# DreamScene-Project/DreamScene

Hardware: AMD Instinct MI355X
Metric: fwd+bwd views/s @1024x1024, 500000 Gaussians (higher is better)
Workload: dtype f32

## Files before the change

### dreamscene_amd/csrc/radix_sort.h

```cpp
#pragma once
#include "gsr_common.h"
#include <type_traits>

namespace {

constexpr int kSortThreads = 256;
constexpr int kItemsLarge = 16;
constexpr int kItemsSmall = 4;
constexpr int kRadixBits = 8;
constexpr int kRadix = 1 << kRadixBits;

template <typename T>
__device__ __forceinline__ T* batch_ptr(T* p, size_t bstride) {
  typedef typename std::conditional<std::is_const<T>::value, const char, char>::type B;
  return p ? reinterpret_cast<T*>(reinterpret_cast<B*>(p) + (size_t)blockIdx.y * bstride) : p;
}
#define GSR_LDS_ORDER() asm volatile("" ::: "memory")

__device__ __forceinline__ uint64_t eff_count(const uint64_t* n_dev, uint64_t cap) {
  if (!n_dev) return cap;
  const uint64_t n = *n_dev;
  return n < cap ? n : cap;
}

template <int ITEMS>
__device__ __forceinline__ uint64_t sort_index(uint32_t blk, int wave, int item, int lane) {
  return (uint64_t)blk * (kSortThreads * ITEMS) + (uint64_t)(wave * (64 * ITEMS) + item * 64 + lane);
}

__device__ __forceinline__ unsigned long long match_digit(uint32_t d, bool valid) {
  unsigned long long m = __ballot(valid);
#pragma unroll
  for (int b = 0; b < kRadixBits; ++b) {
    const bool bit = (d >> b) & 1u;
    const unsigned long long bal = __ballot(bit);
    m &= bit ? bal : ~bal;
  }
  return m;
}

template <int ITEMS, bool DROP>
__global__ void __launch_bounds__(kSortThreads)
k_radix_hist(const uint32_t* __restrict__ keys, const uint64_t* __restrict__ n_dev, uint64_t cap, int shift,
             uint32_t nblk, uint32_t* __restrict__ hist, size_t bstride) {
  keys = batch_ptr(keys, bstride); n_dev = batch_ptr(n_dev, bstride); hist = batch_ptr(hist, bstride);
  __shared__ uint32_t h[kRadix];
  const int tid = threadIdx.x, lane = tid & 63, wave = tid >> 6;
  const uint64_t n = eff_count(n_dev, cap);
  h[tid] = 0;
  __syncthreads();
  if ((uint64_t)blockIdx.x * (kSortThreads * ITEMS) < n) {
#pragma unroll 4
    for (int it = 0; it < ITEMS; ++it) {
      const uint64_t e = sort_index<ITEMS>(blockIdx.x, wave, it, lane);
      bool valid = e < n;
      const uint32_t kk = valid ? keys[e] : 0u;
      if (DROP) valid = valid && (kk != 0xFFFFFFFFu);
      const uint32_t d = (kk >> shift) & (kRadix - 1);
      const unsigned long long m = match_digit(d, valid);
      if (valid && lane == __ffsll((long long)m) - 1) atomicAdd(&h[d], (uint32_t)__popcll(m));
    }
  }
  __syncthreads();
  hist[(uint64_t)tid * nblk + blockIdx.x] = h[tid];
}

template <int THREADS>
__device__ __forceinline__ void radix_scan_body(uint32_t* __restrict__ hist, uint32_t nblk_stride, uint32_t* __restrict__ totals,
                                                const uint64_t* __restrict__ n_items, uint32_t per_block, size_t bstride) {
  hist = batch_ptr(hist, bstride); totals = batch_ptr(totals, bstride); n_items = batch_ptr(n_items, bstride);
  uint32_t nblk = nblk_stride;
  if (n_items) {
    const uint64_t used = (*n_items + per_block - 1) / per_block;
    if (used < nblk) nblk = (uint32_t)used;
  }
  constexpr int NW = THREADS / 64;
  __shared__ uint32_t wave_tot[NW];
  __shared__ uint32_t carry_s;
  const int tid = threadIdx.x, lane = tid & 63, wave = tid >> 6;
  uint32_t* row = hist + (uint64_t)blockIdx.x * nblk_stride;
  if (tid == 0) carry_s = 0;
  __syncthreads();
  constexpr uint32_t kPer = 4;
  for (uint32_t base = 0; base < nblk; base += THREADS * kPer) {
    uint32_t x[kPer];
    uint32_t s = 0;
    const uint32_t first = base + tid * kPer;
#pragma unroll
    for (uint32_t k = 0; k < kPer; ++k) {
      x[k] = (first + k < nblk) ? row[first + k] : 0u;
      s += x[k];
    }
    uint32_t inc = s;
#pragma unroll
    for (int o = 1; o < 64; o <<= 1) {
      const uint32_t t = (uint32_t)__shfl_up((int)inc, o, 64);
      if (lane >= o) inc += t;
    }
    if (lane == 63) wave_tot[wave] = inc;
    __syncthreads();
    uint32_t woff = 0;
#pragma unroll
    for (int w = 0; w < NW; ++w) woff += (w < wave) ? wave_tot[w] : 0u;
    const uint32_t carry = carry_s;
    uint32_t run = carry + woff + inc - s;
#pragma unroll
    for (uint32_t k = 0; k < kPer; ++k) {
      if (first + k < nblk) row[first + k] = run;
      run += x[k];
    }
    __syncthreads();
    if (tid == THREADS - 1) carry_s = carry + woff + inc;
    __syncthreads();
  }
  if (tid == 0) totals[blockIdx.x] = carry_s;
}
__global__ void __launch_bounds__(256) k_radix_scan(uint32_t* __restrict__ hist, uint32_t nblk_stride,
                                                    uint32_t* __restrict__ totals,
                                                    const uint64_t* __restrict__ n_items, uint32_t per_block,
                                                    size_t bstride) {
  radix_scan_body<256>(hist, nblk_stride, totals, n_items, per_block, bstride);
}
__global__ void __launch_bounds__(1024) k_radix_scan_wide(uint32_t* __restrict__ hist, uint32_t nblk_stride,
                                                          uint32_t* __restrict__ totals,
                                                          const uint64_t* __restrict__ n_items, uint32_t per_block,
                                                          size_t bstride) {
  radix_scan_body<1024>(hist, nblk_stride, totals, n_items, per_block, bstride);
}

template <bool IOTA, int ITEMS, bool DROP>
__global__ void __launch_bounds__(kSortThreads)
k_radix_scatter(const uint32_t* __restrict__ keys_in, const uint32_t* __restrict__ vals_in,
                uint32_t* __restrict__ keys_out, uint32_t* __restrict__ vals_out, const uint64_t* __restrict__ n_dev,
                uint64_t cap, int shift, uint32_t nblk, const uint32_t* __restrict__ hist,
                const uint32_t* __restrict__ totals, uint64_t* __restrict__ n_out, size_t bstride) {
  keys_in = batch_ptr(keys_in, bstride); vals_in = batch_ptr(vals_in, bstride);
  keys_out = batch_ptr(keys_out, bstride); vals_out = batch_ptr(vals_out, bstride);
  n_dev = batch_ptr(n_dev, bstride); hist = batch_ptr(hist, bstride); totals = batch_ptr(totals, bstride);
  n_out = batch_ptr(n_out, bstride);
  __shared__ uint32_t wh[4][kRadix];
  __shared__ uint32_t dbase[kRadix];
  __shared__ uint32_t wtot[4];
  const int tid = threadIdx.x, lane = tid & 63, wave = tid >> 6;
  const uint64_t n = eff_count(n_dev, cap);
  if ((uint64_t)blockIdx.x * (kSortThreads * ITEMS) >= n) {
    if (DROP && n_out && blockIdx.x == 0 && tid == 0) *n_out = 0;
    return;
  }
#pragma unroll
  for (int w = 0; w < 4; ++w) wh[w][tid] = 0;
  {
    const uint32_t x = totals[tid];
    uint32_t inc = x;
#pragma unroll
    for (int o = 1; o < 64; o <<= 1) {
      const uint32_t t = (uint32_t)__shfl_up((int)inc, o, 64);
      if (lane >= o) inc += t;
    }
    if (lane == 63) wtot[wave] = inc;
    __syncthreads();
    uint32_t woff = 0;
    for (int w = 0; w < wave; ++w) woff += wtot[w];
    dbase[tid] = woff + inc - x;
    if (DROP && n_out && blockIdx.x == 0 && tid == kSortThreads - 1) *n_out = (uint64_t)(woff + inc);
  }
  __syncthreads();
  uint32_t* mywh = wh[wave];
  uint32_t key[ITEMS];
  uint32_t val[ITEMS];
  uint32_t rank[ITEMS];
  const unsigned long long lt = (1ull << lane) - 1ull;
#pragma unroll
  for (int it = 0; it < ITEMS; ++it) {
    const uint64_t e = sort_index<ITEMS>(blockIdx.x, wave, it, lane);
    const bool valid = e < n;
    key[it] = valid ? keys_in[e] : 0xFFFFFFFFu;
    val[it] = IOTA ? (uint32_t)e : (valid ? vals_in[e] : 0u);
  }
  const auto is_valid = [&](int it) {
    const uint64_t e = sort_index<ITEMS>(blockIdx.x, wave, it, lane);
    return (e < n) && (!DROP || key[it] != 0xFFFFFFFFu);
  };
#pragma unroll
  for (int it = 0; it < ITEMS; ++it) {
    const bool valid = is_valid(it);
    const uint32_t d = (key[it] >> shift) & (kRadix - 1);
    const unsigned long long m = match_digit(d, valid);
    const int leader = __ffsll((long long)m) - 1;
    uint32_t old = 0;
    if (valid && lane == leader) {
      old = mywh[d];
      mywh[d] = old + (uint32_t)__popcll(m);
    }
    old = (uint32_t)__shfl((int)old, valid ? leader : lane, 64);
    rank[it] = old + (uint32_t)__popcll(m & lt);
    GSR_LDS_ORDER();
  }
  __syncthreads();
  {
    uint32_t run = dbase[tid] + hist[(uint64_t)tid * nblk + blockIdx.x];
#pragma unroll
    for (int w = 0; w < 4; ++w) {
      const uint32_t c = wh[w][tid];
      wh[w][tid] = run;
      run += c;
    }
  }
  __syncthreads();
#pragma unroll
  for (int it = 0; it < ITEMS; ++it) {
    if (is_valid(it)) {
      const uint32_t d = (key[it] >> shift) & (kRadix - 1);
      const uint32_t pos = wh[wave][d] + rank[it];
      keys_out[pos] = key[it];
      vals_out[pos] = val[it];
    }
  }
}

#ifndef GSR_OS_ITEMS_SMALL
#define GSR_OS_ITEMS_SMALL 16
#endif
constexpr int kOsItemsSmall = GSR_OS_ITEMS_SMALL;
constexpr int kOsMaxPasses = 4;
#ifndef GSR_OS_HIST_TILE
#define GSR_OS_HIST_TILE 2048
#endif
constexpr uint32_t kOsHistTile = GSR_OS_HIST_TILE;
constexpr uint32_t kOsTableOff = kOsMaxPasses * kRadix + 16;
constexpr uint32_t kOsSkipFlag = kOsMaxPasses * kRadix + 8;
constexpr uint32_t kOsEarlyN = kOsMaxPasses * kRadix + 10;
constexpr uint64_t kOsMaxN = 1ull << 28;

typedef __attribute__((address_space(1))) uint32_t gsr_gu32;
__device__ __forceinline__ gsr_gu32* gsr_global(uint32_t* p) { return (gsr_gu32*)(uintptr_t)p; }

__host__ __device__ inline uint32_t os_tiles(uint64_t n, int items) {
  const uint64_t t = (uint64_t)kSortThreads * items;
  return (uint32_t)((n + t - 1) / t);
}
__host__ inline size_t os_state_words(uint64_t n, int items) { return (size_t)kOsTableOff + (size_t)kRadix * os_tiles(n, items); }

template <bool DROP>
__global__ void __launch_bounds__(kSortThreads)
k_os_hist(const uint32_t* __restrict__ keys, const uint64_t* __restrict__ n_dev, uint64_t cap, int passes,
          uint32_t* __restrict__ os, size_t bstride, const uint32_t* __restrict__ wrect) {
  keys = batch_ptr(keys, bstride); n_dev = batch_ptr(n_dev, bstride); os = batch_ptr(os, bstride);
  wrect = batch_ptr(wrect, bstride);
  __shared__ uint32_t h[kOsMaxPasses][kRadix];
  __shared__ uint32_t wsum[kSortThreads / 64];
  const int tid = threadIdx.x, lane = tid & 63;
  const uint64_t n = eff_count(n_dev, cap);
  const uint64_t base = (uint64_t)blockIdx.x * kOsHistTile;
  if (base >= n) return;
#pragma unroll
  for (int p = 0; p < kOsMaxPasses; ++p) h[p][tid] = 0;
  __syncthreads();
  constexpr int kPer = kOsHistTile / kSortThreads;
  uint32_t kk[kPer];
  uint32_t weight = 0;
#pragma unroll
  for (int it = 0; it < kPer; ++it) {
    const uint64_t e = base + (uint64_t)(it * kSortThreads + tid);
    kk[it] = e < n ? keys[e] : 0xFFFFFFFFu;
    if (wrect && e < n && (!DROP || kk[it] != 0xFFFFFFFFu)) {
      const uint32_t r = wrect[e];
      weight += (((r >> 16) & 255u) + 1u) * ((r >> 24) + 1u);
    }
  }
  if (wrect) {
#pragma unroll
    for (int o = 32; o > 0; o >>= 1) weight += (uint32_t)__shfl_xor((int)weight, o, 64);
    if (lane == 0) wsum[tid >> 6] = weight;
  }
#pragma unroll
  for (int it = 0; it < kPer; ++it) {
    const uint64_t e = base + (uint64_t)(it * kSortThreads + tid);
    const bool valid = (e < n) && (!DROP || kk[it] != 0xFFFFFFFFu);
    const unsigned long long vm = __ballot(valid);
    if (vm == 0ull) continue;
    const uint32_t k = kk[it];
    if (valid) {
      atomicAdd(&h[0][k & (kRadix - 1)], 1u);
      if (passes > 1) atomicAdd(&h[1][(k >> kRadixBits) & (kRadix - 1)], 1u);
    }
    if (passes > 2) {
      const int first = __ffsll((long long)vm) - 1;
      const uint32_t hi = k >> (2 * kRadixBits), hi0 = (uint32_t)__shfl((int)hi, first, 64);
      if (__ballot(valid && hi != hi0) == 0ull) {
        if (lane == first) {
          atomicAdd(&h[2][hi0 & (kRadix - 1)], (uint32_t)__popcll(vm));
          if (passes > 3) atomicAdd(&h[3][hi0 >> kRadixBits], (uint32_t)__popcll(vm));
        }
      } else if (valid) {
        atomicAdd(&h[2][hi & (kRadix - 1)], 1u);
        if (passes > 3) atomicAdd(&h[3][hi >> kRadixBits], 1u);
      }
    }
  }
  __syncthreads();
  for (int p = 0; p < passes; ++p) {
    const uint32_t c = h[p][tid];
    if (c) atomicAdd(&os[p * kRadix + tid], c);
  }
  if (wrect && tid == 0) {
    const uint64_t w = ((uint64_t)wsum[0] + wsum[1]) + ((uint64_t)wsum[2] + wsum[3]);
    if (w) atomicAdd(reinterpret_cast<unsigned long long*>(os + kOsEarlyN), (unsigned long long)w);
  }
}

#ifndef GSR_OS_WINDOW
#define GSR_OS_WINDOW 16
#endif
constexpr int kOsWindow = GSR_OS_WINDOW;
__device__ __forceinline__ uint32_t os_look_back(gsr_gu32* table, uint32_t tile, int col, uint32_t tagA, uint32_t tagI) {
  uint32_t excl = 0;
  int p = (int)tile - 1;
  for (;;) {
    uint32_t w[kOsWindow];
#pragma unroll
    for (int j = 0; j < kOsWindow; ++j)
      w[j] = (p - j >= 0) ? __hip_atomic_load(table + (size_t)(p - j) * kRadix + col, __ATOMIC_RELAXED, __HIP_MEMORY_SCOPE_AGENT)
                          : 0u;
    bool done = false, stalled = false;
#pragma unroll
    for (int j = 0; j < kOsWindow; ++j) {
      if (done || stalled) continue;
      const uint32_t tag = w[j] & 0xF0000000u;
      if (tag == tagI) { excl += w[j] & 0x0FFFFFFFu; done = true; }
      else if (tag == tagA) { excl += w[j] & 0x0FFFFFFFu; --p; }
      else stalled = true;
    }
    if (done) return excl;
    if (stalled) __builtin_amdgcn_s_sleep(1);
  }
}

#ifdef GSR_OS_TRACE
__device__ unsigned long long* g_os_trace = nullptr;
#define GSR_OS_STAMP(k) do { if (threadIdx.x == 0 && g_os_trace) \
    g_os_trace[(((size_t)pass * 4 + blockIdx.y) * 4096 + blockIdx.x) * 8 + (k)] = wall_clock64(); } while (0)
#else
#define GSR_OS_STAMP(k) do { } while (0)
#endif

template <bool IOTA, int ITEMS, bool DROP>
__global__ void __launch_bounds__(kSortThreads)
k_os_pass(const uint32_t* __restrict__ keys_in, const uint32_t* __restrict__ vals_in, uint32_t* __restrict__ keys_out,
          uint32_t* __restrict__ vals_out, const uint64_t* __restrict__ n_dev, uint64_t cap, int pass,
          uint32_t* __restrict__ os, uint64_t* __restrict__ n_out, size_t bstride, const int may_skip,
          uint64_t* __restrict__ early_out) {
  keys_in = batch_ptr(keys_in, bstride); vals_in = batch_ptr(vals_in, bstride);
  keys_out = batch_ptr(keys_out, bstride); vals_out = batch_ptr(vals_out, bstride);
  n_dev = batch_ptr(n_dev, bstride); os = batch_ptr(os, bstride); n_out = batch_ptr(n_out, bstride);
  constexpr uint32_t T = kSortThreads * ITEMS;
  __shared__ uint32_t wh[4][kRadix];
  __shared__ uint32_t gbase[kRadix];
  __shared__ uint32_t skey[T], sval[T];
  __shared__ uint32_t wtot[4];
  __shared__ uint32_t s_tile, s_ntile;
  const int tid = threadIdx.x, lane = tid & 63, wave = tid >> 6;
  const int shift = pass * kRadixBits;
  const uint64_t n = eff_count(n_dev, cap);
  if constexpr (!DROP) {
    const uint32_t x = os[pass * kRadix + tid];
    if (__syncthreads_or((uint64_t)x == n && n > 0)) {
      if (may_skip) {
        if (blockIdx.x == 0 && tid == 0) os[kOsSkipFlag] = 1u;
        return;
      }
#pragma unroll
      for (int it = 0; it < ITEMS; ++it) {
        const uint64_t e = sort_index<ITEMS>(blockIdx.x, wave, it, lane);
        if (e < n) {
          keys_out[e] = keys_in[e];
          vals_out[e] = IOTA ? (uint32_t)e : vals_in[e];
        }
      }
      return;
    }
  }
  GSR_OS_STAMP(0);
  if (tid == 0) s_tile = atomicAdd(&os[kOsMaxPasses * kRadix + pass], 1u);
#pragma unroll
  for (int w = 0; w < 4; ++w) wh[w][tid] = 0;
  __syncthreads();
  const uint32_t tile = s_tile;
  if (early_out && tile == 0 && tid == 0)
    __hip_atomic_store(early_out + blockIdx.y, *reinterpret_cast<const uint64_t*>(os + kOsEarlyN), __ATOMIC_RELAXED,
                       __HIP_MEMORY_SCOPE_SYSTEM);
  if ((uint64_t)tile * T >= n) {
    if (DROP && n_out && tile == 0 && tid == 0) *n_out = 0;
    return;
  }
  uint32_t dbase;
  {
    const uint32_t x = os[pass * kRadix + tid];
    uint32_t inc = x;
#pragma unroll
    for (int o = 1; o < 64; o <<= 1) {
      const uint32_t t = (uint32_t)__shfl_up((int)inc, o, 64);
      if (lane >= o) inc += t;
    }
    if (lane == 63) wtot[wave] = inc;
    __syncthreads();
    uint32_t woff = 0;
    for (int w = 0; w < wave; ++w) woff += wtot[w];
    dbase = woff + inc - x;
    if (DROP && n_out && tile == 0 && tid == kSortThreads - 1) *n_out = (uint64_t)(woff + inc);
  }
  GSR_OS_STAMP(1);
#ifdef GSR_OS_TRACE
  if (threadIdx.x == 0 && g_os_trace) g_os_trace[(((size_t)pass * 4 + blockIdx.y) * 4096 + blockIdx.x) * 8 + 7] = tile;
#endif
  uint32_t* mywh = wh[wave];
  uint32_t key[ITEMS], val[ITEMS], rank[ITEMS];
  const unsigned long long lt = (1ull << lane) - 1ull;
#pragma unroll
  for (int it = 0; it < ITEMS; ++it) {
    const uint64_t e = sort_index<ITEMS>(tile, wave, it, lane);
    const bool valid = e < n;
    key[it] = valid ? keys_in[e] : 0xFFFFFFFFu;
    val[it] = IOTA ? (uint32_t)e : (valid ? vals_in[e] : 0u);
  }
  const auto is_valid = [&](int it) {
    const uint64_t e = sort_index<ITEMS>(tile, wave, it, lane);
    return (e < n) && (!DROP || key[it] != 0xFFFFFFFFu);
  };
#pragma unroll
  for (int it = 0; it < ITEMS; ++it) {
    const bool valid = is_valid(it);
    const uint32_t d = (key[it] >> shift) & (kRadix - 1);
    const unsigned long long m = match_digit(d, valid);
    const int leader = __ffsll((long long)m) - 1;
    uint32_t old = 0;
    if (valid && lane == leader) {
      old = mywh[d];
      mywh[d] = old + (uint32_t)__popcll(m);
    }
    old = (uint32_t)__shfl((int)old, valid ? leader : lane, 64);
    rank[it] = old + (uint32_t)__popcll(m & lt);
    GSR_LDS_ORDER();
  }
  __syncthreads();
  GSR_OS_STAMP(2);
  uint32_t cnt;
  {
    uint32_t run = 0;
#pragma unroll
    for (int w = 0; w < 4; ++w) {
      const uint32_t c = wh[w][tid];
      wh[w][tid] = run;
      run += c;
    }
    cnt = run;
  }
  gsr_gu32* table = gsr_global(os + kOsTableOff);
  const uint32_t tagA = (uint32_t)(2 * pass + 1) << 28, tagI = (uint32_t)(2 * pass + 2) << 28;
  uint32_t excl = 0;
  if (tile == 0) {
    __hip_atomic_store(table + tid, tagI | cnt, __ATOMIC_RELAXED, __HIP_MEMORY_SCOPE_AGENT);
  } else {
    __hip_atomic_store(table + (size_t)tile * kRadix + tid, tagA | cnt, __ATOMIC_RELAXED, __HIP_MEMORY_SCOPE_AGENT);
    excl = os_look_back(table, tile, tid, tagA, tagI);
    __hip_atomic_store(table + (size_t)tile * kRadix + tid, tagI | (excl + cnt), __ATOMIC_RELAXED, __HIP_MEMORY_SCOPE_AGENT);
  }
  GSR_OS_STAMP(3);
  uint32_t lstart;
  {
    uint32_t inc = cnt;
#pragma unroll
    for (int o = 1; o < 64; o <<= 1) {
      const uint32_t t = (uint32_t)__shfl_up((int)inc, o, 64);
      if (lane >= o) inc += t;
    }
    __syncthreads();
    if (lane == 63) wtot[wave] = inc;
    __syncthreads();
    uint32_t woff = 0;
    for (int w = 0; w < wave; ++w) woff += wtot[w];
    lstart = woff + inc - cnt;
    if (tid == kSortThreads - 1) s_ntile = woff + inc;
  }
#pragma unroll
  for (int w = 0; w < 4; ++w) wh[w][tid] += lstart;
  gbase[tid] = dbase + excl - lstart;
  __syncthreads();
#pragma unroll
  for (int it = 0; it < ITEMS; ++it) {
    if (is_valid(it)) {
      const uint32_t d = (key[it] >> shift) & (kRadix - 1);
      const uint32_t lp = wh[wave][d] + rank[it];
      skey[lp] = key[it];
      sval[lp] = val[it];
    }
  }
  __syncthreads();
  GSR_OS_STAMP(4);
  const uint32_t ntile = s_ntile;
  for (uint32_t i = tid; i < ntile; i += kSortThreads) {
    const uint32_t k = skey[i];
    const uint32_t pos = gbase[(k >> shift) & (kRadix - 1)] + i;
    keys_out[pos] = k;
    vals_out[pos] = sval[i];
  }
  GSR_OS_STAMP(5);
}

__host__ inline size_t align256(size_t x) { return (x + 255) & ~(size_t)255; }

uint32_t sort_blocks(uint64_t n, int items) {
  const uint64_t t = (uint64_t)kSortThreads * items;
  return (uint32_t)((n + t - 1) / t);
}

__host__ inline size_t sort_hist_bytes(uint64_t n, int items_legacy, int items_os) {
  const size_t legacy = (size_t)kRadix * sort_blocks(n, items_legacy) * 4;
  const size_t os = os_state_words(n, items_os) * 4;
  return align256(legacy > os ? legacy : os);
}

template <int ITEMS>
int radix_sort_u32_legacy(uint32_t* k0, uint32_t* v0, uint32_t* k1, uint32_t* v1, const uint64_t* n_dev, uint64_t cap,
                          int bits, bool iota, uint64_t* n_compact, uint32_t* hist, uint32_t* totals, hipStream_t stream,
                          int batch = 1, size_t bstride = 0);

template <int ITEMS, int OS_ITEMS>
int radix_sort_u32(uint32_t* k0, uint32_t* v0, uint32_t* k1, uint32_t* v1, const uint64_t* n_dev, uint64_t cap,
                   int bits, bool iota, uint64_t* n_compact, uint32_t* hist, uint32_t* totals, hipStream_t stream,
                   int batch = 1, size_t bstride = 0, bool state_cleared = false, bool last_pass_may_skip = false,
                   const uint32_t* early_rects = nullptr, uint64_t* early_out = nullptr) {
  const int passes = (bits + kRadixBits - 1) / kRadixBits;
  if (cap >= kOsMaxN || passes > kOsMaxPasses)
    return radix_sort_u32_legacy<ITEMS>(k0, v0, k1, v1, n_dev, cap, bits, iota, n_compact, hist, totals, stream, batch, bstride);
  const uint32_t ntile = os_tiles(cap, OS_ITEMS), nhist = (uint32_t)((cap + kOsHistTile - 1) / kOsHistTile);
  const dim3 grid(ntile, (uint32_t)batch), grid_h(nhist ? nhist : 1, (uint32_t)batch);
  if (!state_cleared &&
      gsr_zero_async(hist, os_state_words(cap, OS_ITEMS) * 4, stream, bstride, (uint32_t)batch) != hipSuccess) return passes & 1;
  const bool drop = iota && n_compact;
  if (!drop) { early_rects = nullptr; early_out = nullptr; }
  if (!early_out) early_rects = nullptr;
  if (drop)
    hipLaunchKernelGGL((k_os_hist<true>), grid_h, dim3(kSortThreads), 0, stream, k0, n_dev, cap, passes, hist, bstride,
                       early_rects);
  else
    hipLaunchKernelGGL((k_os_hist<false>), grid_h, dim3(kSortThreads), 0, stream, k0, n_dev, cap, passes, hist, bstride,
                       (const uint32_t*)nullptr);
  uint32_t *ka = k0, *va = v0, *kb = k1, *vb = v1;
  for (int p = 0; p < passes; ++p) {
    if (p == 0 && drop) {
      hipLaunchKernelGGL((k_os_pass<true, OS_ITEMS, true>), grid, dim3(kSortThreads), 0, stream, ka, va, kb, vb, n_dev, cap, p,
                         hist, n_compact, bstride, 0, early_rects ? early_out : (uint64_t*)nullptr);
      n_dev = n_compact;
    } else if (p == 0 && iota) {
      hipLaunchKernelGGL((k_os_pass<true, OS_ITEMS, false>), grid, dim3(kSortThreads), 0, stream, ka, va, kb, vb, n_dev, cap, p,
                         hist, (uint64_t*)nullptr, bstride, 0, (uint64_t*)nullptr);
    } else {
      hipLaunchKernelGGL((k_os_pass<false, OS_ITEMS, false>), grid, dim3(kSortThreads), 0, stream, ka, va, kb, vb, n_dev, cap, p,
                         hist, (uint64_t*)nullptr, bstride, (last_pass_may_skip && p == passes - 1 && p > 0) ? 1 : 0,
                         (uint64_t*)nullptr);
    }
    uint32_t* t = ka; ka = kb; kb = t;
    t = va; va = vb; vb = t;
  }
  return passes & 1;
}

template <int ITEMS>
int radix_sort_u32_legacy(uint32_t* k0, uint32_t* v0, uint32_t* k1, uint32_t* v1, const uint64_t* n_dev, uint64_t cap,
                   int bits, bool iota, uint64_t* n_compact, uint32_t* hist, uint32_t* totals, hipStream_t stream,
                   int batch, size_t bstride) {
  const uint32_t nblk = sort_blocks(cap, ITEMS);
  const int passes = (bits + kRadixBits - 1) / kRadixBits;
  const dim3 grid(nblk, (uint32_t)batch), grid_scan(kRadix, (uint32_t)batch);
  uint32_t *ka = k0, *va = v0, *kb = k1, *vb = v1;
  for (int p = 0; p < passes; ++p) {
    const int shift = p * kRadixBits;
    if (iota && p == 0 && n_compact) {
      hipLaunchKernelGGL((k_radix_hist<ITEMS, true>), grid, dim3(kSortThreads), 0, stream, ka, n_dev, cap, shift, nblk,
                         hist, bstride);
      hipLaunchKernelGGL(k_radix_scan, grid_scan, dim3(256), 0, stream, hist, nblk, totals, (const uint64_t*)nullptr, 1u,
                         bstride);
      hipLaunchKernelGGL((k_radix_scatter<true, ITEMS, true>), grid, dim3(kSortThreads), 0, stream, ka, va, kb, vb, n_dev,
                         cap, shift, nblk, hist, totals, n_compact, bstride);
      n_dev = n_compact;
    } else {
      hipLaunchKernelGGL((k_radix_hist<ITEMS, false>), grid, dim3(kSortThreads), 0, stream, ka, n_dev, cap, shift, nblk,
                         hist, bstride);
      hipLaunchKernelGGL(k_radix_scan, grid_scan, dim3(256), 0, stream, hist, nblk, totals, (const uint64_t*)nullptr, 1u,
                         bstride);
      if (iota && p == 0)
        hipLaunchKernelGGL((k_radix_scatter<true, ITEMS, false>), grid, dim3(kSortThreads), 0, stream, ka, va, kb, vb,
                           n_dev, cap, shift, nblk, hist, totals, (uint64_t*)nullptr, bstride);
      else
        hipLaunchKernelGGL((k_radix_scatter<false, ITEMS, false>), grid, dim3(kSortThreads), 0, stream, ka, va, kb, vb,
                           n_dev, cap, shift, nblk, hist, totals, (uint64_t*)nullptr, bstride);
    }
    uint32_t* t = ka; ka = kb; kb = t;
    t = va; va = vb; vb = t;
  }
  return passes & 1;
}

}
```

Baseline: 5121.

## Publish onesweep tile counts early and widen histogram blocks for batched sorts

The onesweep pass kernel now loads its keys first and builds per-tile digit counts in shared memory with atomics. It publishes the aggregate to the look-back table before the full per-wave ranking, so later tiles spin less on the decoupled look-back. The histogram kernel is templated on thread count and tile size, and batched sorts (batch>=2) use 1024-thread blocks over 8192-element tiles. This cuts block count and global atomics, at the cost of an extra LDS atomic pass per tile and more shared memory.

```diff
diff --git a/dreamscene_amd/csrc/radix_sort.h b/dreamscene_amd/csrc/radix_sort.h
--- a/dreamscene_amd/csrc/radix_sort.h
+++ b/dreamscene_amd/csrc/radix_sort.h
@@ -227,6 +227,12 @@
 #define GSR_OS_HIST_TILE 2048
 #endif
 constexpr uint32_t kOsHistTile = GSR_OS_HIST_TILE;
+#ifndef GSR_OS_HIST_WIDE
+#define GSR_OS_HIST_WIDE 1
+#endif
+constexpr int kOsHistWideThreads = 1024;
+constexpr uint32_t kOsHistWideTile = 8192;
+__host__ inline bool os_hist_wide(int batch) { return GSR_OS_HIST_WIDE && batch >= 2; }
 constexpr uint32_t kOsTableOff = kOsMaxPasses * kRadix + 16;
 constexpr uint32_t kOsSkipFlag = kOsMaxPasses * kRadix + 8;
 constexpr uint32_t kOsEarlyN = kOsMaxPasses * kRadix + 10;
@@ -241,27 +247,29 @@
 }
 __host__ inline size_t os_state_words(uint64_t n, int items) { return (size_t)kOsTableOff + (size_t)kRadix * os_tiles(n, items); }
 
-template <bool DROP>
-__global__ void __launch_bounds__(kSortThreads)
+template <bool DROP, int THREADS = kSortThreads, uint32_t TILE = kOsHistTile>
+__global__ void __launch_bounds__(THREADS)
 k_os_hist(const uint32_t* __restrict__ keys, const uint64_t* __restrict__ n_dev, uint64_t cap, int passes,
           uint32_t* __restrict__ os, size_t bstride, const uint32_t* __restrict__ wrect) {
   keys = batch_ptr(keys, bstride); n_dev = batch_ptr(n_dev, bstride); os = batch_ptr(os, bstride);
   wrect = batch_ptr(wrect, bstride);
   __shared__ uint32_t h[kOsMaxPasses][kRadix];
-  __shared__ uint32_t wsum[kSortThreads / 64];
+  __shared__ uint32_t wsum[THREADS / 64];
   const int tid = threadIdx.x, lane = tid & 63;
   const uint64_t n = eff_count(n_dev, cap);
-  const uint64_t base = (uint64_t)blockIdx.x * kOsHistTile;
+  const uint64_t base = (uint64_t)blockIdx.x * TILE;
   if (base >= n) return;
-#pragma unroll
-  for (int p = 0; p < kOsMaxPasses; ++p) h[p][tid] = 0;
-  __syncthreads();
-  constexpr int kPer = kOsHistTile / kSortThreads;
+  if (tid < kRadix) {
+#pragma unroll
+    for (int p = 0; p < kOsMaxPasses; ++p) h[p][tid] = 0;
+  }
+  __syncthreads();
+  constexpr int kPer = TILE / THREADS;
   uint32_t kk[kPer];
   uint32_t weight = 0;
 #pragma unroll
   for (int it = 0; it < kPer; ++it) {
-    const uint64_t e = base + (uint64_t)(it * kSortThreads + tid);
+    const uint64_t e = base + (uint64_t)(it * THREADS + tid);
     kk[it] = e < n ? keys[e] : 0xFFFFFFFFu;
     if (wrect && e < n && (!DROP || kk[it] != 0xFFFFFFFFu)) {
       const uint32_t r = wrect[e];
@@ -275,7 +283,7 @@
   }
 #pragma unroll
   for (int it = 0; it < kPer; ++it) {
-    const uint64_t e = base + (uint64_t)(it * kSortThreads + tid);
+    const uint64_t e = base + (uint64_t)(it * THREADS + tid);
     const bool valid = (e < n) && (!DROP || kk[it] != 0xFFFFFFFFu);
     const unsigned long long vm = __ballot(valid);
     if (vm == 0ull) continue;
@@ -299,18 +307,25 @@
     }
   }
   __syncthreads();
-  for (int p = 0; p < passes; ++p) {
-    const uint32_t c = h[p][tid];
-    if (c) atomicAdd(&os[p * kRadix + tid], c);
+  if (tid < kRadix) {
+    for (int p = 0; p < passes; ++p) {
+      const uint32_t c = h[p][tid];
+      if (c) atomicAdd(&os[p * kRadix + tid], c);
+    }
   }
   if (wrect && tid == 0) {
-    const uint64_t w = ((uint64_t)wsum[0] + wsum[1]) + ((uint64_t)wsum[2] + wsum[3]);
+    uint64_t w = 0;
+#pragma unroll
+    for (int i = 0; i < THREADS / 64; ++i) w += wsum[i];
     if (w) atomicAdd(reinterpret_cast<unsigned long long*>(os + kOsEarlyN), (unsigned long long)w);
   }
 }
 
 #ifndef GSR_OS_WINDOW
 #define GSR_OS_WINDOW 16
+#endif
+#ifndef GSR_OS_EARLY_PUBLISH
+#define GSR_OS_EARLY_PUBLISH 1
 #endif
 constexpr int kOsWindow = GSR_OS_WINDOW;
 __device__ __forceinline__ uint32_t os_look_back(gsr_gu32* table, uint32_t tile, int col, uint32_t tagA, uint32_t tagI) {
@@ -359,6 +374,9 @@
   __shared__ uint32_t skey[T], sval[T];
   __shared__ uint32_t wtot[4];
   __shared__ uint32_t s_tile, s_ntile;
+#if GSR_OS_EARLY_PUBLISH
+  __shared__ uint32_t tcnt[kRadix];
+#endif
   const int tid = threadIdx.x, lane = tid & 63, wave = tid >> 6;
   const int shift = pass * kRadixBits;
   const uint64_t n = eff_count(n_dev, cap);
@@ -384,6 +402,9 @@
   if (tid == 0) s_tile = atomicAdd(&os[kOsMaxPasses * kRadix + pass], 1u);
 #pragma unroll
   for (int w = 0; w < 4; ++w) wh[w][tid] = 0;
+#if GSR_OS_EARLY_PUBLISH
+  tcnt[tid] = 0;
+#endif
   __syncthreads();
   const uint32_t tile = s_tile;
   if (early_out && tile == 0 && tid == 0)
@@ -393,6 +414,25 @@
     if (DROP && n_out && tile == 0 && tid == 0) *n_out = 0;
     return;
   }
+  uint32_t* mywh = wh[wave];
+  uint32_t key[ITEMS], val[ITEMS], rank[ITEMS];
+  const unsigned long long lt = (1ull << lane) - 1ull;
+#pragma unroll
+  for (int it = 0; it < ITEMS; ++it) {
+    const uint64_t e = sort_index<ITEMS>(tile, wave, it, lane);
+    const bool valid = e < n;
+    key[it] = valid ? keys_in[e] : 0xFFFFFFFFu;
+    val[it] = IOTA ? (uint32_t)e : (valid ? vals_in[e] : 0u);
+  }
+  const auto is_valid = [&](int it) {
+    const uint64_t e = sort_index<ITEMS>(tile, wave, it, lane);
+    return (e < n) && (!DROP || key[it] != 0xFFFFFFFFu);
+  };
+#if GSR_OS_EARLY_PUBLISH
+#pragma unroll
+  for (int it = 0; it < ITEMS; ++it)
+    if (is_valid(it)) atomicAdd(&tcnt[(key[it] >> shift) & (kRadix - 1)], 1u);
+#endif
   uint32_t dbase;
   {
     const uint32_t x = os[pass * kRadix + tid];
@@ -413,20 +453,15 @@
 #ifdef GSR_OS_TRACE
   if (threadIdx.x == 0 && g_os_trace) g_os_trace[(((size_t)pass * 4 + blockIdx.y) * 4096 + blockIdx.x) * 8 + 7] = tile;
 #endif
-  uint32_t* mywh = wh[wave];
-  uint32_t key[ITEMS], val[ITEMS], rank[ITEMS];
-  const unsigned long long lt = (1ull << lane) - 1ull;
-#pragma unroll
-  for (int it = 0; it < ITEMS; ++it) {
-    const uint64_t e = sort_index<ITEMS>(tile, wave, it, lane);
-    const bool valid = e < n;
-    key[it] = valid ? keys_in[e] : 0xFFFFFFFFu;
-    val[it] = IOTA ? (uint32_t)e : (valid ? vals_in[e] : 0u);
-  }
-  const auto is_valid = [&](int it) {
-    const uint64_t e = sort_index<ITEMS>(tile, wave, it, lane);
-    return (e < n) && (!DROP || key[it] != 0xFFFFFFFFu);
-  };
+  gsr_gu32* table = gsr_global(os + kOsTableOff);
+  const uint32_t tagA = (uint32_t)(2 * pass + 1) << 28, tagI = (uint32_t)(2 * pass + 2) << 28;
+#if !GSR_OS_EARLY_PUBLISH
+  uint32_t cnt;
+#else
+  const uint32_t cnt = tcnt[tid];
+  __hip_atomic_store(table + (size_t)tile * kRadix + tid, (tile == 0 ? tagI : tagA) | cnt, __ATOMIC_RELAXED,
+                     __HIP_MEMORY_SCOPE_AGENT);
+#endif
 #pragma unroll
   for (int it = 0; it < ITEMS; ++it) {
     const bool valid = is_valid(it);
@@ -444,7 +479,6 @@
   }
   __syncthreads();
   GSR_OS_STAMP(2);
-  uint32_t cnt;
   {
     uint32_t run = 0;
 #pragma unroll
@@ -453,15 +487,19 @@
       wh[w][tid] = run;
       run += c;
     }
+#if !GSR_OS_EARLY_PUBLISH
     cnt = run;
-  }
-  gsr_gu32* table = gsr_global(os + kOsTableOff);
-  const uint32_t tagA = (uint32_t)(2 * pass + 1) << 28, tagI = (uint32_t)(2 * pass + 2) << 28;
+#endif
+  }
   uint32_t excl = 0;
+#if !GSR_OS_EARLY_PUBLISH
   if (tile == 0) {
     __hip_atomic_store(table + tid, tagI | cnt, __ATOMIC_RELAXED, __HIP_MEMORY_SCOPE_AGENT);
   } else {
     __hip_atomic_store(table + (size_t)tile * kRadix + tid, tagA | cnt, __ATOMIC_RELAXED, __HIP_MEMORY_SCOPE_AGENT);
+  }
+#endif
+  if (tile != 0) {
     excl = os_look_back(table, tile, tid, tagA, tagI);
     __hip_atomic_store(table + (size_t)tile * kRadix + tid, tagI | (excl + cnt), __ATOMIC_RELAXED, __HIP_MEMORY_SCOPE_AGENT);
   }
@@ -533,16 +571,24 @@
   const int passes = (bits + kRadixBits - 1) / kRadixBits;
   if (cap >= kOsMaxN || passes > kOsMaxPasses)
     return radix_sort_u32_legacy<ITEMS>(k0, v0, k1, v1, n_dev, cap, bits, iota, n_compact, hist, totals, stream, batch, bstride);
-  const uint32_t ntile = os_tiles(cap, OS_ITEMS), nhist = (uint32_t)((cap + kOsHistTile - 1) / kOsHistTile);
+  const bool hist_wide = os_hist_wide(batch);
+  const uint32_t hist_tile = hist_wide ? kOsHistWideTile : kOsHistTile;
+  const uint32_t ntile = os_tiles(cap, OS_ITEMS), nhist = (uint32_t)((cap + hist_tile - 1) / hist_tile);
   const dim3 grid(ntile, (uint32_t)batch), grid_h(nhist ? nhist : 1, (uint32_t)batch);
   if (!state_cleared &&
       gsr_zero_async(hist, os_state_words(cap, OS_ITEMS) * 4, stream, bstride, (uint32_t)batch) != hipSuccess) return passes & 1;
   const bool drop = iota && n_compact;
   if (!drop) { early_rects = nullptr; early_out = nullptr; }
   if (!early_out) early_rects = nullptr;
-  if (drop)
+  if (drop && hist_wide)
+    hipLaunchKernelGGL((k_os_hist<true, kOsHistWideThreads, kOsHistWideTile>), grid_h, dim3(kOsHistWideThreads), 0, stream, k0,
+                       n_dev, cap, passes, hist, bstride, early_rects);
+  else if (drop)
     hipLaunchKernelGGL((k_os_hist<true>), grid_h, dim3(kSortThreads), 0, stream, k0, n_dev, cap, passes, hist, bstride,
                        early_rects);
+  else if (hist_wide)
+    hipLaunchKernelGGL((k_os_hist<false, kOsHistWideThreads, kOsHistWideTile>), grid_h, dim3(kOsHistWideThreads), 0, stream, k0,
+                       n_dev, cap, passes, hist, bstride, (const uint32_t*)nullptr);
   else
     hipLaunchKernelGGL((k_os_hist<false>), grid_h, dim3(kSortThreads), 0, stream, k0, n_dev, cap, passes, hist, bstride,
                        (const uint32_t*)nullptr);
```

Result: no change. 5167 (median of 6 runs) (+0.9%).
